# mlozhechko/course5

Measured on AMD Instinct MI355X. Metric: Mrays/sec at 2400x1800 on 1M-tet grid, higher is better.
Workload: dtype f64

## Files before the change

### course5_amd/build.py

```python
from __future__ import annotations

import os
import shutil
import subprocess
import sys

PKG = os.path.dirname(os.path.abspath(__file__))
CSRC = os.path.join(PKG, "csrc")
OUT = os.path.join(PKG, "_build")
LIB = os.path.join(PKG, "libcourse5_hip.so")
CLI = os.path.join(PKG, "course")
ARCH = "gfx950"

HIPCC = shutil.which("hipcc") or "/opt/rocm/bin/hipcc"
COMMON = ["-O3", "-std=c++17", "-fPIC", f"--offload-arch={ARCH}", "-Wall", "-Wextra",
          "-Wno-unused-parameter", "-I", os.path.join(PKG, "..", "include")]

LIB_SOURCES = [
    ("exact_kernels.hip", ["-ffp-contract=off"]),
    ("walk_kernels.hip", []),
    ("adjoint_kernels.hip", ["-munsafe-fp-atomics"]),
    ("context.hip", []),
    ("grid.hip", []),
    ("frame.hip", []),
    ("derivatives.hip", []),
    ("host_ring.hip", []),
    ("adjacency.cpp", ["-x", "c++", "-fopenmp"]),
]


DEVICE_SOURCES = ("device_types.hpp", "kernels.hpp", "walk_common.hpp", "exact_kernels.hip", "walk_kernels.hip")


def kernel_source_hash() -> str:
    import hashlib
    import re
    h = hashlib.sha256()
    for name in DEVICE_SOURCES:
        with open(os.path.join(CSRC, name)) as f:
            text = f.read()
        text = re.sub(r"/\*.*?\*/", "", text, flags=re.S)
        text = re.sub(r"//[^\n]*", "", text)
        h.update(name.encode())
        h.update("".join(text.split()).encode())
    return h.hexdigest()[:16]


def _newer(target: str, deps: list[str]) -> bool:
    if not os.path.exists(target):
        return True
    t = os.path.getmtime(target)
    return any(os.path.getmtime(d) > t for d in deps if os.path.exists(d))


def _run(cmd: list[str], verbose: bool) -> None:
    if verbose:
        print(" ".join(cmd), flush=True)
    subprocess.run(cmd, check=True)


def build_library(verbose: bool = False, force: bool = False) -> str:
    os.makedirs(OUT, exist_ok=True)
    headers = [os.path.join(CSRC, h) for h in os.listdir(CSRC) if h.endswith((".hpp", ".h"))]
    headers.append(os.path.join(PKG, "..", "include", "course5_hip.h"))
    objs = []
    for src, extra in LIB_SOURCES:
        s = os.path.join(CSRC, src)
        o = os.path.join(OUT, os.path.splitext(src)[0] + ".o")
        if force or _newer(o, [s] + headers):
            _run([HIPCC] + COMMON + extra + ["-c", s, "-o", o], verbose)
        objs.append(o)
    if force or _newer(LIB, objs):
        _run([HIPCC, "-shared", "-fPIC", f"--offload-arch={ARCH}", "-o", LIB] + objs + ["-fopenmp"], verbose)
# ... 26 lines not shown
```

### course5_amd/csrc/context.hip

```cpp
#include "context.hpp"

namespace c5api __attribute__((visibility("hidden"))) {

namespace {
std::string g_create_error;
}

int fail(c5_context* ctx, int code, const char* fmt, ...) {
    char buf[512];
    va_list ap;
    va_start(ap, fmt);
    vsnprintf(buf, sizeof buf, fmt, ap);
    va_end(ap);
    if (ctx)
        ctx->error = buf;
    else
        g_create_error = buf;
    return code;
}

int bind_device(c5_context* ctx) {
    C5_HIP(ctx, hipSetDevice(ctx->device));
    return C5_OK;
}
// ... 472 lines not shown
    if (!ctx) return fail(nullptr, C5_ERR_INVALID, "null context");
    ctx->alpha_limit = alpha_limit;
    return C5_OK;
}

int c5_set_option(c5_context* ctx, const char* name, double value) {
    if (!ctx || !name) return fail(ctx, C5_ERR_INVALID, "null option");
    const std::string n(name);
    if (n != "row_costs" && n != "stage_timing" && n != "walk_timing") ++ctx->setup_epoch;
    if (n == "tile") {
        if (value < 0 || value > 3) return fail(ctx, C5_ERR_INVALID, "tile must be 0, 1, 2 or 3");
        ctx->tile_shape = static_cast<int>(value);
    } else if (n == "transmittance_cutoff") {
        ctx->t_cutoff = value;
    } else if (n == "pipeline") {
        int rc = bind_device(ctx);
        if (rc) return rc;
        rc = drain(ctx);
        if (rc) return rc;
        if (ctx->n_cells > 0 || ctx->have_image)
            return fail(ctx, C5_ERR_STATE, "set \"pipeline\" before uploading the grid and setting the image");
        ctx->pipeline = static_cast<int>(value) != 0;
    } else if (n == "fuse_setup") {
        ctx->fuse_setup = static_cast<int>(value) != 0;
    } else if (n == "overlap_setup") {
        ctx->overlap_setup = static_cast<int>(value) != 0;
    } else if (n == "cell_order") {
        ctx->cell_order = static_cast<int>(value) != 0;
    } else if (n == "block_cull") {
        ctx->block_cull = static_cast<int>(value) != 0;
    } else if (n == "tile_flags") {
        ctx->tile_flags = static_cast<int>(value) != 0;
    } else if (n == "cost_order") {
        ctx->cost_order = static_cast<int>(value);
    } else if (n == "entry_key") {
        ctx->entry_key = static_cast<int>(value) != 0;
        ctx->overlap_seen = false;
    } else if (n == "stage_slots") {
        if (value != 0 && value != 14 && value != 21) return fail(ctx, C5_ERR_INVALID, "stage_slots must be 0 (per frame), 14 or 21");
        ctx->stage_slots = static_cast<int>(value);
    } else if (n == "solid_interior_faces") {
        ctx->solid_interior_faces = static_cast<int>(value) != 0;
        forget_solid_masks(ctx);
    } else if (n == "view_cache") {
        ctx->view_cache = static_cast<int>(value) != 0;
    } else if (n == "batch_width") {
        if (value != 0 && value != 4 && value != 8) return fail(ctx, C5_ERR_INVALID, "batch_width must be 0 (by the batch), 4 or 8");
        ctx->batch_width = static_cast<int>(value);
    } else if (n == "vertex_merge") {
        ctx->vertex_merge = static_cast<int>(value) != 0;
    } else if (n == "split_tilt_x" || n == "split_tilt_y") {
        if (!(std::fabs(value) < 64.0)) return fail(ctx, C5_ERR_INVALID, "split tilt out of range");
        (n == "split_tilt_x" ? ctx->split_tilt_x : ctx->split_tilt_y) = value;
    } else if (n == "entry_records") {
        ctx->entry_records = static_cast<int>(value) != 0;
    } else if (n == "depth_split") {
        if (value < 0 || value > c5::kMaxSlabs || value != std::floor(value))
            return fail(ctx, C5_ERR_INVALID, "depth_split must be 0 (per frame), 1 (never) or 2..%d slabs", c5::kMaxSlabs);
        ctx->depth_split = static_cast<int>(value);
    } else if (n == "solid_cache") {
        ctx->solid_cache = static_cast<int>(value) != 0;
        forget_solid_masks(ctx);
    } else if (n == "algorithm") {
        if (value != 0 && value != 1) return fail(ctx, C5_ERR_INVALID, "algorithm must be 0 (walk) or 1 (bin_sort_resolve)");
        ctx->algorithm = static_cast<int>(value);
    } else if (n == "lds_stage") {
        ctx->lds_stage = static_cast<int>(value) < 0 ? 0 : (static_cast<int>(value) > 2 ? 2 : static_cast<int>(value));
    } else if (n == "integration") {
        ctx->order = static_cast<int>(value) != 0;
    } else if (n == "entry_pool") {
        if (value < 1 || value > 16777214) return fail(ctx, C5_ERR_INVALID, "entry_pool out of range");
        int rc = drain(ctx);
        if (rc) return rc;
        for (FrameSlot& fs : ctx->slots) {
            fs.entry_capacity = static_cast<int64_t>(value);
            C5_HIP(ctx, fs.pool.ensure(static_cast<size_t>(fs.entry_capacity) * sizeof(c5::Entry)));
        }
    } else if (n == "band_rows") {
        if (value < 0 || value > 4096) return fail(ctx, C5_ERR_INVALID, "band_rows out of range");
        ctx->band_rows = static_cast<int>(value);
    } else if (n == "lds_pad") {
        if (value < 0 || value > 96 * 1024) return fail(ctx, C5_ERR_INVALID, "lds_pad out of range");
        ctx->lds_pad = static_cast<int>(value);
    } else if (n == "xcd_mode") {
        ctx->xcd_mode = static_cast<int>(value) < 0 ? 0 : (static_cast<int>(value) > 2 ? 2 : static_cast<int>(value));
    } else if (n == "row_costs") {
        ctx->row_costs = static_cast<int>(value) != 0;
    } else if (n == "stage_timing") {
        ctx->stage_timing = static_cast<int>(value) != 0;
    } else if (n == "walk_timing") {
        if (!(value >= 0.0 && value <= 1024.0)) return fail(ctx, C5_ERR_INVALID, "walk_timing: 0 (off) or every N-th launch, N <= 1024");
        ctx->walk_timing = static_cast<int>(value);
        ctx->walk_seq = 0;
    } else {
        return fail(ctx, C5_ERR_INVALID, "unknown option '%s'", name);
    }
    return C5_OK;
}

int c5_get_stats(c5_context* ctx, c5_stats* out) {
    if (!ctx || !out) return fail(ctx, C5_ERR_INVALID, "null argument");
    int rc = c5_synchronize(ctx);
    *out = ctx->last;
    return rc;
}

// ... 67 lines not shown
```

### course5_amd/csrc/context.hpp

```cpp
#pragma once
#include <hip/hip_runtime.h>

#include <algorithm>

#include <cfloat>
#include <cmath>
#include <cstdarg>
#include <cstddef>
#include <cstdio>
#include <cstring>
#include <new>
#include <string>
#include <vector>

#include "../../include/course5_hip.h"
#include "adjacency.hpp"
#include "adjoint.hpp"
#include "device_types.hpp"
#include "kernels.hpp"

namespace c5api __attribute__((visibility("hidden"))) {

struct DeviceBuffer {
    void* ptr = nullptr;
    size_t bytes = 0;
    hipError_t ensure(size_t want) {
        if (want <= bytes && ptr) return hipSuccess;
        if (ptr) {
            hipError_t e = hipFree(ptr);
            ptr = nullptr;
            bytes = 0;
            if (e != hipSuccess) return e;
        }
        if (want == 0) return hipSuccess;
        hipError_t e = hipMalloc(&ptr, want);
        if (e == hipSuccess) bytes = want;
        return e;
    }
    void release() {
        if (ptr) (void)hipFree(ptr);
        ptr = nullptr;
        bytes = 0;
    }
    template <class T>
    T* as() const {
        return static_cast<T*>(ptr);
    }
};

struct Solid {
    int64_t n_tets = 0;
    int64_t n_points = 0;
    int64_t n_faces = 0;
    int64_t n_interior = 0;
    double colour = 0.0;
    struct FaceGroup {
        int64_t begin, count;
        double longest;
    };
    std::vector<FaceGroup> groups;
    double centre[3] = {0, 0, 0};
    double radius = 0.0;
    DeviceBuffer raw;
    DeviceBuffer faces;
    DeviceBuffer view[2];
    c5::RotationList rots{};
    DeviceBuffer own_mask;
    c5::RotationList seen_rots{};
    c5::ImageParams seen_im{};
    uint64_t generation = 0, seen_generation = ~uint64_t{0};
    hipStream_t seen_stream = nullptr;
    int unchanged_frames = 0;
    bool own_mask_ready = false;
};

inline bool same_rotations(const c5::RotationList& a, const c5::RotationList& b) {
    if (a.n != b.n) return false;
    for (int k = 0; k < a.n; ++k)
        if (a.axis[k] != b.axis[k] || a.cosv[k] != b.cosv[k] || a.sinv[k] != b.sinv[k] || a.x0[k] != b.x0[k]) return false;
    return true;
}
inline bool same_image(const c5::ImageParams& a, const c5::ImageParams& b) {
    return a.res_x == b.res_x && a.res_y == b.res_y && a.n_local_rows == b.n_local_rows && a.tile_rows == b.tile_rows &&
           a.rank == b.rank && a.world == b.world && a.row_begin == b.row_begin && a.row_count == b.row_count &&
           a.x_min == b.x_min && a.y_min == b.y_min && a.step_x == b.step_x && a.step_y == b.step_y;
}

constexpr int kWalkEventPool = 512;
constexpr size_t kStageChunk = size_t{4} << 20;
constexpr int kFrameSlots = 2;
constexpr int kStickyWords = 3;
constexpr int kStatusWords = 3;
constexpr int64_t kMaxEntryPool = int64_t{16777214} * 64;
constexpr size_t kCountersBytes = sizeof(c5::FrameCounters) * c5::kCounterLines;

struct FrameSlot {
    DeviceBuffer vx, vy, vz, rec, count, head, first, pool, mask, counters, row_cost;
    DeviceBuffer sb;
    long long sb_key = -1;
    int sb_n = 0;
    uint64_t setup_epoch = 0;
    c5::RotationList setup_view{};
    double setup_limit = 0.0;
    int setup_order = 0;
    bool setup_kept = false;
    bool setup_reused = false;
    const c5::FrameCounters* raster_counters = nullptr;
    DeviceBuffer plane_cell, straddle, straddle_count, partials, arrivals;
    DeviceBuffer bfrec;
    uint32_t bf_seq = 0;
    int split_k = 0;
    int64_t split_px = 0, split_tiles = 0, split_cells = 0;
    uint64_t split_seq = 0;
    int setup_split = 1;
    double setup_w[c5::kMaxSlabs + 1] = {};
    double setup_g[2] = {0.0, 0.0};
    int64_t entry_capacity = 0;
    DeviceBuffer tile_flag;
    uint32_t flag_seq = 0;
    int64_t flag_tiles = 0;
    bool flags_valid = false;
    bool head_clean = false;
    c5::FrameCounters* host_counters = nullptr;
    hipEvent_t setup_done = nullptr, walk_done = nullptr;
    bool walk_recorded = false;
    hipEvent_t ev[7] = {nullptr, nullptr, nullptr, nullptr, nullptr, nullptr, nullptr};
};

}

struct c5_context {
    int device = 0;
    hipStream_t stream = nullptr;
    hipStream_t own_stream = nullptr;
    std::string error;

    int64_t n_pts = 0, n_cells = 0, n_bfaces = 0;
    hipStream_t aux_stream = nullptr;
    hipStream_t side_stream = nullptr;
    hipEvent_t fork_ev = nullptr, join_ev = nullptr;
    int fuse_setup = 0;
    int cell_order = 1;
    std::vector<int32_t> cell_perm;
    int block_cull = 1;
    int tile_flags = 1;
    int cost_order = 1;
    uint8_t sb_order[128] = {};
    long long sb_order_key = -1;
    int sb_order_n = 0;
    uint32_t* host_sb = nullptr;
    int entry_key = 1;
    int stage_slots = 0;
    double rays_per_cell = 0.0;
    int solid_cache = 1;
    int view_cache = 1;
    uint64_t setup_epoch = 1;
    int solid_interior_faces = 0;
    int depth_split = 0;
    int entry_records = 1;
    int split_auto_k = 1;
    bool ray_depth_known = false;
    double ray_depth_lo = 0.0, ray_depth_hi = 0.0;
    bool fit_known = false;
    double fit_gx = 0.0, fit_gy = 0.0, fit_entry0 = 0.0, fit_exit0 = 0.0;
    double split_tilt_x = 0.0, split_tilt_y = 0.0;
    double box_lo[3] = {0, 0, 0}, box_hi[3] = {0, 0, 0};
    double alpha_floor = 0.0;
    int overlap_setup = 0;
    c5api::DeviceBuffer px, py, pz, cell_vert, cell_adj, alpha, q, bface, block_sphere;
    double alpha_top = 0.0;
    double edge_max = 0.0;
    double grid_diagonal = 0.0;
    double coord_max = 0.0;
    c5api::FrameSlot slots[c5api::kFrameSlots];
    int64_t frame_index = 0;
    int last_slot = 0;
    void* last_counters = nullptr;
    int row_cost_slot = 0;
    int algorithm = 0;
    bool grid_conforming = true;
    bool overlap_seen = false;
    c5api::DeviceBuffer offs64, scratch64, segs;
    int pipeline = 0;
    c5::RotationList view{};
    c5api::Solid solids[C5_MAX_SOLIDS];

    bool have_image = false;
    double bounds[4] = {0, 0, 0, 0};
    c5::ImageParams im{};
    int cfg_tile_rows = 0, cfg_rank = 0, cfg_world = 1;
    int cfg_row_begin = 0, cfg_row_count = -1;
    c5api::DeviceBuffer xtab, ytab, out, sticky;
    unsigned* host_sticky = nullptr;
    std::vector<double> host_ytab;
    int row_costs = 0;
    bool row_costs_collected = false;

    double alpha_limit = 2.5;
    double t_cutoff = 1e-12;
    int tile_shape = 3;
    int xcd_mode = 2;
    int lds_pad = 0;
    int band_rows = 0;
    int order = 0;
    int lds_stage = 2;
    int stage_timing = 0;
    int walk_timing = 0;
    unsigned walk_seq = 0;

    hipEvent_t walk_a[c5api::kWalkEventPool];
    hipEvent_t walk_b[c5api::kWalkEventPool];
    int walk_used = 0;
    double walk_ms_sum = 0.0;
    int64_t walk_launches = 0;

    struct HostFrame {
        c5api::DeviceBuffer img;
        c5api::DeviceBuffer counters;
        hipEvent_t rendered = nullptr, copied = nullptr;
        unsigned* status = nullptr;
    };
    hipStream_t copy_stream = nullptr;
// ... 15 lines not shown
    c5api::DeviceBuffer adj_grad;
    c5api::DeviceBuffer adj_perm;
    uint64_t grid_serial = 0, adj_perm_serial = ~uint64_t{0};
    unsigned* adj_status = nullptr;
    bool adjoint_pending = false;
    const char* adj_what = "adjoint";

    c5api::DeviceBuffer tan_dir;

    int batch_width = 0;
    c5api::DeviceBuffer bat_dirs;
    c5api::DeviceBuffer bat_grad;
    c5api::DeviceBuffer gn_g;
    c5api::DeviceBuffer gn_spare;
    c5api::DeviceBuffer vtx_face;
    c5api::DeviceBuffer vtx_grad;
    int vertex_merge = 1;
    c5api::DeviceBuffer vtx_vel;
    std::vector<int32_t> host_cell_vert, point_rep;
    c5api::DeviceBuffer deriv_io;
    c5api::DeviceBuffer scal_stats;
    unsigned long long* scal_host = nullptr;
};

namespace c5api __attribute__((visibility("hidden"))) {

int fail(c5_context* ctx, int code, const char* fmt, ...);

#define C5_HIP(ctx, expr)                                                                        \
    do {                                                                                         \
        hipError_t e_ = (expr);                                                                  \
        if (e_ != hipSuccess)                                                                    \
            return fail((ctx), C5_ERR_HIP, "%s failed: %s (%s:%d)", #expr, hipGetErrorString(e_), \
                        __FILE__, __LINE__);                                                     \
    } while (0)

int bind_device(c5_context* ctx);
int to_rotation_list(c5_context* ctx, const c5_rotation* rots, int n, c5::RotationList& out);
void rotate_host(const c5::RotationList& R, double c[3]);
int drain(c5_context* ctx);
int grow_entry_pools(c5_context* ctx, int64_t want);

int ensure_device_perm(c5_context* ctx);

inline int64_t local_pixels(const c5::ImageParams& im) { return static_cast<int64_t>(im.n_local_rows) * im.res_x; }
inline int64_t padded_pixels(const c5::ImageParams& im) { return ((local_pixels(im) + 1023) / 1024) * 1024; }
inline size_t image_bytes(const c5_context* ctx) { return static_cast<size_t>(local_pixels(ctx->im)) * 2 * sizeof(float); }
bool nothing_to_render(const c5_context* ctx);
bool uses_bin_sort(const c5_context* ctx);
double entry_key_slack(const c5_context* ctx);
c5::GridView grid_view(const c5_context* ctx, const FrameSlot& fs);
int enqueue_bin_lists(c5_context* ctx, FrameSlot& fs, const c5::GridView& g, hipStream_t s, c5::FrameCounters* counters, int64_t& total);
int enqueue_solids(c5_context* ctx, FrameSlot& fs, int slot_id, hipStream_t s, c5::SolidTable& table, bool& any_solid);
int enqueue_frame(c5_context* ctx, float2* out_dev, c5::FrameCounters* own_counters = nullptr);
int wait_and_collect(c5_context* ctx);

int finish_adjoint(c5_context* ctx);

}
```

### course5_amd/csrc/derivatives.hip

```cpp
#include "context.hpp"

using namespace c5api;

namespace {

struct DerivativeView {
    bool no_cells = false;
    bool bin_sort = false;
    hipStream_t s = nullptr;
    int64_t n_px = 0, padded = 0;
    const int32_t* perm = nullptr;
    c5::GridView g{};
    const uint32_t* mask = nullptr;
    c5::WalkParams w{};
};

int setup_derivative(c5_context* ctx, DerivativeView& v) {
    if (nothing_to_render(ctx)) return fail(ctx, C5_ERR_STATE, "plane initializer. empty set of objects to render");
    if (!ctx->have_image) return fail(ctx, C5_ERR_STATE, "critical error. empty plane");
    int rc = bind_device(ctx);
    if (rc) return rc;
    FrameSlot& fs = ctx->slots[0];
    hipStream_t s = v.s = ctx->stream;
    const c5::ImageParams& im = ctx->im;
    v.n_px = local_pixels(im);
    const int64_t padded = v.padded = padded_pixels(im);
    if (ctx->n_cells <= 0) {
        v.no_cells = true;
        return C5_OK;
    }
    if (c5::segment_bytes() != c5::adjoint_segment_bytes())
        return fail(ctx, C5_ERR_STATE, "bin_sort_resolve's segment layout differs from the adjoint's");
    if (ctx->pipeline || ctx->overlap_setup) {
        rc = drain(ctx);
        if (rc) return rc;
    }

    C5_HIP(ctx, ctx->adj_counters.ensure(kCountersBytes));
    C5_HIP(ctx, ctx->adj_sticky.ensure(kStickyWords * sizeof(unsigned)));
    if (!ctx->adj_status) C5_HIP(ctx, hipHostMalloc(reinterpret_cast<void**>(&ctx->adj_status), 4 * sizeof(unsigned), hipHostMallocDefault));
    rc = ensure_device_perm(ctx);
    if (rc) return rc;
    v.perm = ctx->cell_perm.empty() ? nullptr : ctx->adj_perm.as<int32_t>();
    c5::FrameCounters* const counters = ctx->adj_counters.as<c5::FrameCounters>();
    C5_HIP(ctx, hipMemsetAsync(ctx->adj_sticky.ptr, 0, kStickyWords * sizeof(unsigned), s));

    c5::GridView& g = v.g = grid_view(ctx, fs);
    fs.setup_epoch = 0;
    fs.setup_kept = false;
    fs.flags_valid = false;

    c5::launch_transform_soa(s, g.px, g.py, g.pz, g.vx, g.vy, g.vz, g.n_pts, ctx->view, counters);
    c5::SolidTable table{};
    bool any_solid = false;
    v.bin_sort = uses_bin_sort(ctx);
    if (v.bin_sort) {
        int64_t total = 0;
        rc = enqueue_bin_lists(ctx, fs, g, s, counters, total);
        if (rc) return rc;
        rc = enqueue_solids(ctx, fs, 0, s, table, any_solid);
        if (rc) return rc;
        v.mask = any_solid ? fs.mask.as<uint32_t>() : nullptr;
    } else {
        const double key_slack = entry_key_slack(ctx);
        c5::launch_build_records(s, g, ctx->alpha_limit, 0);
        if (!fs.head_clean) C5_HIP(ctx, hipMemsetAsync(fs.head.ptr, 0, static_cast<size_t>(padded) * sizeof(c5::EntryHead), s));
        fs.head_clean = false;
        c5::launch_entry_lists(s, g, ctx->xtab.as<double>(), ctx->ytab.as<double>(), im, fs.head.as<c5::EntryHead>(),
                               fs.first.as<c5::Entry>(), fs.pool.as<c5::Entry>(), fs.entry_capacity, counters,
                               ctx->adj_sticky.as<unsigned>(), 0, key_slack);
        rc = enqueue_solids(ctx, fs, 0, s, table, any_solid);
        if (rc) return rc;
        v.mask = any_solid ? fs.mask.as<uint32_t>() : nullptr;
        c5::WalkParams& wp = v.w;
        wp.xrec = g.xrec;
        wp.entry_head = fs.head.as<c5::EntryHead>();
        wp.entry_first = fs.first.as<c5::Entry>();
        wp.entry_pool = fs.pool.as<c5::Entry>();
        wp.pool_capacity = fs.entry_capacity;
        wp.key_slack = key_slack > 0.0 ? key_slack : 0.0;
        wp.mask = v.mask;
        wp.solids = table;
        wp.Xtab = ctx->xtab.as<double>();
        wp.Ytab = ctx->ytab.as<double>();
        wp.im = im;
        wp.max_steps = static_cast<uint32_t>(ctx->n_cells + 64);
        wp.counters = counters;
        wp.sticky = ctx->adj_sticky.as<unsigned>();
    }
    return C5_OK;
}

int commit_derivative(c5_context* ctx, const char* what) {
    FrameSlot& fs = ctx->slots[0];
    hipStream_t s = ctx->stream;
    C5_HIP(ctx, hipGetLastError());
    C5_HIP(ctx, hipMemcpyAsync(ctx->adj_status, &ctx->adj_counters.as<c5::FrameCounters>()->walk_overflow,
                               kStatusWords * sizeof(unsigned), hipMemcpyDeviceToHost, s));
    if (ctx->pipeline) {
        C5_HIP(ctx, hipEventRecord(fs.walk_done, s));
        fs.walk_recorded = true;
    }
    ctx->adjoint_pending = true;
    ctx->adj_what = what;
    return C5_OK;
}

int adjoint_params(c5_context* ctx, const DerivativeView& v, c5::AdjointParams& ap) {
    C5_HIP(ctx, ctx->adj_lambda.ensure(static_cast<size_t>(v.padded) * sizeof(double)));
    ap = c5::AdjointParams{};
    ap.w = v.w;
    ap.lambda = ctx->adj_lambda.as<double>();
    return C5_OK;
}

int adjoint_one(c5_context* ctx, const DerivativeView& v, bool squared, const float2* weights, double* ga_out, double* gq_out) {
    const size_t n_cells = static_cast<size_t>(ctx->n_cells);
    C5_HIP(ctx, ctx->adj_grad.ensure(2 * n_cells * sizeof(double)));
// ... 613 lines not shown
```

### course5_amd/csrc/frame.hip

```cpp
#include "context.hpp"

namespace c5api __attribute__((visibility("hidden"))) {

constexpr double kSplitAlphaFloor = 1e-6;

int enqueue_solids(c5_context* ctx, FrameSlot& fs, int slot_id, hipStream_t s, c5::SolidTable& table, bool& any_solid) {
    const c5::ImageParams& im = ctx->im;
    const int64_t padded = padded_pixels(im);
    any_solid = false;
    for (int k = 0; k < C5_MAX_SOLIDS; ++k) {
        table.colour[k] = ctx->solids[k].colour;
        if (ctx->solids[k].n_tets > 0) any_solid = true;
    }
    table.n_slots = C5_MAX_SOLIDS;
    if (any_solid) {
        C5_HIP(ctx, hipMemsetAsync(fs.mask.ptr, 0, static_cast<size_t>(padded) * sizeof(uint32_t), s));
        for (int k = 0; k < C5_MAX_SOLIDS; ++k) {
            Solid& so = ctx->solids[k];
            if (so.n_tets <= 0) continue;
            const bool same = ctx->solid_cache && !ctx->pipeline && so.seen_stream == s && so.seen_generation == so.generation &&
                              same_rotations(so.seen_rots, so.rots) && same_image(so.seen_im, im);
            so.unchanged_frames = same ? so.unchanged_frames + 1 : 0;
            if (!same) {
                so.own_mask_ready = false;
// ... 130 lines not shown
    fs.host_counters->seg_tiles = static_cast<unsigned long long>(total);
    if (ctx->pipeline) {
        C5_HIP(ctx, hipEventRecord(fs.setup_done, s));
        C5_HIP(ctx, hipStreamWaitEvent(f.main_s, fs.setup_done, 0));
        C5_HIP(ctx, hipEventRecord(fs.walk_done, f.main_s));
        fs.walk_recorded = true;
    }
    note_enqueued(ctx, f);
    return C5_OK;
}

}

bool nothing_to_render(const c5_context* ctx) {
    if (ctx->n_cells > 0) return false;
    for (const Solid& s : ctx->solids)
        if (s.n_tets > 0) return false;
    return true;
}

c5::GridView grid_view(const c5_context* ctx, const FrameSlot& fs) {
    const c5::ImageParams& im = ctx->im;
    c5::GridView g;
    g.n_pts = ctx->n_pts;
    g.n_cells = ctx->n_cells;
    g.n_bfaces = ctx->n_bfaces;
    g.px = ctx->px.as<double>();
    g.py = ctx->py.as<double>();
    g.pz = ctx->pz.as<double>();
    g.vx = fs.vx.as<double>();
    g.vy = fs.vy.as<double>();
    g.vz = fs.vz.as<double>();
    g.cell_vert = ctx->cell_vert.as<int4>();
    g.cell_adj = ctx->cell_adj.as<int4>();
    g.alpha = ctx->alpha.as<double>();
    g.q = ctx->q.as<double>();
    g.bface = ctx->bface.as<uint32_t>();
    g.xrec = fs.rec.as<c5::ExitRecord>();
    g.rot = ctx->view;
    g.block_sphere = (ctx->block_cull && im.n_local_rows > 0 && im.n_local_rows < im.res_y && ctx->block_sphere.ptr) ? ctx->block_sphere.as<double4>() : nullptr;
    if (im.n_local_rows > 0) {
        const int first = c5::global_row_of(im, 0), last = c5::global_row_of(im, im.n_local_rows - 1);
        const double pad = std::fabs(im.step_y);
        const double ya = ctx->host_ytab[static_cast<size_t>(first)], yb = ctx->host_ytab[static_cast<size_t>(last)];
        g.cull_y_lo = std::fmin(ya, yb) - pad;
        g.cull_y_hi = std::fmax(ya, yb) + pad;
    } else {
        g.cull_y_lo = 1.0;
        g.cull_y_hi = -1.0;
    }
    return g;
}

namespace {


bool serial_setup(const c5_context* ctx) { return !ctx->pipeline && !ctx->fuse_setup && !ctx->overlap_setup; }

bool default_walk(const c5_context* ctx) {
    return ctx->tile_shape == 3 && ctx->xcd_mode == 2 && ctx->lds_stage == 2 && ctx->order == 0;
}

int sb_cost_buffer(c5_context* ctx, FrameJob& f) {
    const c5::ImageParams& im = ctx->im;
    FrameSlot& fs = f.fs;
    if (ctx->cost_order && ctx->xcd_mode == 2 && ctx->lds_stage && im.n_local_rows > 0) {
        const int sb_rows = c5::walk_sb_rows(ctx->tile_shape, ctx->band_rows);
        f.n_sb = (im.n_local_rows + sb_rows - 1) / sb_rows;
        if (f.n_sb <= c5::kMaxSbRows) {
            if (!fs.sb.ptr) {
                C5_HIP(ctx, fs.sb.ensure(c5::kMaxSbRows * sizeof(uint32_t)));
                C5_HIP(ctx, hipMemsetAsync(fs.sb.ptr, 0, fs.sb.bytes, f.s));
            }
            f.sb_key = (static_cast<long long>(im.n_local_rows) << 20) ^ (static_cast<long long>(sb_rows) << 4) ^ ctx->tile_shape;
            f.sb = fs.sb.as<uint32_t>();
        } else {
            f.n_sb = 0;
        }
    }
    fs.sb_key = f.sb_key;
    fs.sb_n = f.n_sb;
    return C5_OK;
}

struct SplitPlan {
    int k = 1;
    double w[c5::kMaxSlabs + 1] = {};
    double g[2] = {0.0, 0.0};
};

void box_depth_range(const c5_context* ctx, const double g[2], double& lo, double& hi) {
    lo = INFINITY, hi = -INFINITY;
    for (int corner = 0; corner < 8; ++corner) {
        double c[3] = {(corner & 1) ? ctx->box_hi[0] : ctx->box_lo[0], (corner & 2) ? ctx->box_hi[1] : ctx->box_lo[1],
                       (corner & 4) ? ctx->box_hi[2] : ctx->box_lo[2]};
        rotate_host(ctx->view, c);
        const double d = c[2] - g[0] * c[0] - g[1] * c[1];
        lo = std::fmin(lo, d);
        hi = std::fmax(hi, d);
    }
}

SplitPlan plan_depth_split(const c5_context* ctx, bool bin_sort) {
    SplitPlan p;
    const bool able = !bin_sort && serial_setup(ctx) && default_walk(ctx) && ctx->n_cells > 0 &&
                      ctx->n_cells < (int64_t{1} << 25) && ctx->im.n_local_rows > 0;
// ... 111 lines not shown
        C5_HIP(ctx, hipMemsetAsync(fs.bfrec.ptr, 0, fs.bfrec.bytes, f.s));
        fs.bf_seq = 0;
    }
    fs.bf_seq += 1;
    if (fs.bf_seq == 0) {
        C5_HIP(ctx, hipMemsetAsync(fs.bfrec.ptr, 0, fs.bfrec.bytes, f.s));
        fs.bf_seq = 1;
    }
    g.bfrec = fs.bfrec.as<c5::BFaceRecord>();
    g.bf_seq = fs.bf_seq;
    g.bf_want_upper = ctx->order != 0;
    g.bf_key_slack = f.key_slack;
    return C5_OK;
}

int tile_flag_buffer(c5_context* ctx, FrameJob& f, const c5::GridView& g, bool fused, hipStream_t e, uint32_t*& tile_flag) {
    FrameSlot& fs = f.fs;
    fs.flags_valid = false;
    if (!(ctx->tile_flags && ctx->tile_shape == 3 && ctx->lds_stage && !fused && g.n_cells > 0 && g.n_bfaces > 0)) return C5_OK;
    const int64_t tiles = c5::walk_tiles(ctx->im);
    if (fs.flag_tiles != tiles || !fs.tile_flag.ptr) {
        C5_HIP(ctx, fs.tile_flag.ensure(static_cast<size_t>(tiles) * sizeof(uint32_t)));
        C5_HIP(ctx, hipMemsetAsync(fs.tile_flag.ptr, 0, static_cast<size_t>(tiles) * sizeof(uint32_t), e));
        fs.flag_tiles = tiles;
        fs.flag_seq = 0;
    }
    fs.flag_seq += 1;
    if (fs.flag_seq == 0) {
        C5_HIP(ctx, hipMemsetAsync(fs.tile_flag.ptr, 0, static_cast<size_t>(tiles) * sizeof(uint32_t), e));
        fs.flag_seq = 1;
    }
    tile_flag = fs.tile_flag.as<uint32_t>();
    fs.flags_valid = true;
    return C5_OK;
}

int enqueue_view_setup(c5_context* ctx, FrameJob& f, c5::GridView& g) {
    FrameSlot& fs = f.fs;
    const c5::ImageParams& im = ctx->im;
    hipStream_t s = f.s;
    const bool side = ctx->overlap_setup && !f.timed;
    hipStream_t e = side ? ctx->side_stream : s;
    if (side) {
        C5_HIP(ctx, hipEventRecord(ctx->fork_ev, s));
        C5_HIP(ctx, hipStreamWaitEvent(e, ctx->fork_ev, 0));
    }
    f.key_slack = entry_key_slack(ctx);
    const bool fused = ctx->fuse_setup && !side && g.n_cells > 0;
    if (!fused && !f.reuse) {
        if (ctx->entry_records && !ctx->fuse_setup && !side && g.n_bfaces > 0) {
            int rc = boundary_records(ctx, f, g);
            if (rc) return rc;
        }
        c5::launch_build_records(s, g, ctx->alpha_limit, ctx->order);
        c5::launch_plane_raster(s, g, ctx->xtab.as<double>(), ctx->ytab.as<double>(), im);
    }
    if (!fused) C5_HIP(ctx, mark(f, 2, s));
    if (!fs.head_clean && !f.reuse) C5_HIP(ctx, hipMemsetAsync(fs.head.ptr, 0, static_cast<size_t>(f.padded) * sizeof(c5::EntryHead), e));
    fs.head_clean = false;
    uint32_t* tile_flag = nullptr;
    if (!f.reuse) {
        int rc = tile_flag_buffer(ctx, f, g, fused, e, tile_flag);
        if (rc) return rc;
    }
    if (fused) {
        c5::launch_setup_fused(s, g, ctx->alpha_limit, ctx->order, ctx->xtab.as<double>(), ctx->ytab.as<double>(), im,
                               fs.head.as<c5::EntryHead>(), fs.first.as<c5::Entry>(), fs.pool.as<c5::Entry>(), fs.entry_capacity,
                               f.counters, ctx->sticky.as<unsigned>(), ctx->order != 0, f.key_slack);
        C5_HIP(ctx, mark(f, 2, s));
    } else if (g.n_cells > 0 && !f.reuse) {
        c5::launch_entry_lists(e, g, ctx->xtab.as<double>(), ctx->ytab.as<double>(), im, fs.head.as<c5::EntryHead>(),
                               fs.first.as<c5::Entry>(), fs.pool.as<c5::Entry>(), fs.entry_capacity, f.counters,
                               ctx->sticky.as<unsigned>(), ctx->order != 0, f.key_slack, tile_flag, fs.flag_seq);
    }
    C5_HIP(ctx, mark(f, 3, e));
    int rc = enqueue_solids(ctx, fs, f.slot_id, e, f.table, f.any_solid);
    if (rc) return rc;
    C5_HIP(ctx, mark(f, 4, e));
    if (side) {
        C5_HIP(ctx, hipEventRecord(ctx->join_ev, e));
        C5_HIP(ctx, hipStreamWaitEvent(s, ctx->join_ev, 0));
    }
    return C5_OK;
}

void fill_walk_params(const c5_context* ctx, const FrameJob& f, const c5::GridView& g, float2* out_dev, c5::WalkParams& wp) {
    const FrameSlot& fs = f.fs;
    wp.xrec = g.xrec;
    wp.entry_head = fs.head.as<c5::EntryHead>();
    wp.entry_first = fs.first.as<c5::Entry>();
    wp.entry_pool = fs.pool.as<c5::Entry>();
    wp.pool_capacity = fs.entry_capacity;
    wp.key_slack = f.key_slack > 0.0 ? f.key_slack : 0.0;
    wp.mask = f.any_solid ? fs.mask.as<uint32_t>() : nullptr;
    wp.solids = f.table;
    wp.Xtab = ctx->xtab.as<double>();
    wp.Ytab = ctx->ytab.as<double>();
    wp.out = out_dev;
    wp.im = ctx->im;
    wp.t_cutoff = ctx->t_cutoff;
    wp.max_steps = static_cast<uint32_t>(ctx->n_cells + 64);
    wp.xcd_mode = ctx->xcd_mode;
    wp.lds_pad = ctx->lds_pad;
    wp.stage_slots = ctx->stage_slots ? ctx->stage_slots : (ctx->rays_per_cell > 0.0 && ctx->rays_per_cell < 120.0 ? 21 : 14);
    wp.band_rows = ctx->band_rows;
    wp.order = ctx->order;
    wp.lds_stage = (ctx->lds_stage && ctx->n_cells < (int64_t{1} << 25)) ? ctx->lds_stage : 0;
    wp.counters = f.counters;
    wp.tile_flag = (fs.flags_valid && !f.any_solid && ctx->tile_flags) ? fs.tile_flag.as<uint32_t>() : nullptr;
    wp.tile_stamp = fs.flag_seq;
    {
        double a_max = std::fmin(ctx->alpha_top, ctx->alpha_limit);
        if (!(a_max >= 0.0)) a_max = ctx->alpha_top;
        wp.small_exp_only = (a_max * ctx->edge_max < 0.125) ? 1 : 0;
    }
    wp.keep_entries = fs.setup_kept ? 1 : 0;
    wp.split = g.split;
    wp.row_cost = nullptr;
    wp.sb_cost = f.sb;
    wp.n_sb_rows = 0;
    if (f.sb && ctx->sb_order_key == f.sb_key && ctx->sb_order_n == f.n_sb) {
// ... 341 lines not shown
```

### course5_amd/csrc/grid.hip

```cpp
#include "context.hpp"

using namespace c5api;

namespace c5api __attribute__((visibility("hidden"))) {

int ensure_device_perm(c5_context* ctx) {
    if (!ctx->cell_perm.empty() && ctx->adj_perm_serial != ctx->grid_serial) {
        const size_t n_cells = static_cast<size_t>(ctx->n_cells);
        C5_HIP(ctx, ctx->adj_perm.ensure(n_cells * sizeof(int32_t)));
        C5_HIP(ctx, hipMemcpy(ctx->adj_perm.ptr, ctx->cell_perm.data(), n_cells * sizeof(int32_t), hipMemcpyHostToDevice));
        ctx->adj_perm_serial = ctx->grid_serial;
    }
    return C5_OK;
}

}

namespace {

void weld_cells(const double* xyz, int64_t n_pts, int64_t n_cells, const int32_t*& cell_vert, std::vector<int32_t>& welded,
                std::vector<int32_t>& rep) {
    if (c5::weld_points(xyz, n_pts, rep) <= 0) {
        rep.clear();
        return;
// ... 123 lines not shown
    for (int64_t i = 0; i < n_pts; ++i)
        for (int k = 0; k < 3; ++k) {
            const double v = xyz[3 * i + k];
            lo[k] = i ? std::fmin(lo[k], v) : v;
            hi[k] = i ? std::fmax(hi[k], v) : v;
            top = std::fmax(top, std::fabs(v));
        }
    for (int k = 0; k < 3; ++k) ctx->box_lo[k] = lo[k], ctx->box_hi[k] = hi[k];
    ctx->grid_diagonal = std::sqrt((hi[0] - lo[0]) * (hi[0] - lo[0]) + (hi[1] - lo[1]) * (hi[1] - lo[1]) + (hi[2] - lo[2]) * (hi[2] - lo[2]));
    ctx->coord_max = top + 2.0;
    double edge2 = 0.0;
    for (int64_t c = 0; c < n_cells; ++c) {
        const int32_t* v = cell_vert + 4 * c;
        for (int a = 0; a < 4; ++a)
            for (int b = a + 1; b < 4; ++b) {
                const double* pa = xyz + 3 * static_cast<int64_t>(v[a]);
                const double* pb = xyz + 3 * static_cast<int64_t>(v[b]);
                const double d2 = (pa[0] - pb[0]) * (pa[0] - pb[0]) + (pa[1] - pb[1]) * (pa[1] - pb[1]) + (pa[2] - pb[2]) * (pa[2] - pb[2]);
                if (d2 > edge2) edge2 = d2;
            }
    }
    ctx->edge_max = std::sqrt(edge2) * (1.0 + 1e-9);
}

int upload_block_spheres(c5_context* ctx, const double* xyz, const int32_t* cell_vert, int64_t n_cells) {
    const int64_t n_blocks = (n_cells + 255) / 256;
    std::vector<double> sph(static_cast<size_t>(4 * n_blocks), 0.0);
    for (int64_t b = 0; b < n_blocks; ++b) {
        double lo[3] = {INFINITY, INFINITY, INFINITY}, hi[3] = {-INFINITY, -INFINITY, -INFINITY};
        for (int64_t c = 256 * b; c < std::min<int64_t>(n_cells, 256 * (b + 1)); ++c)
            for (int a = 0; a < 4; ++a) {
                const double* p = xyz + 3 * static_cast<int64_t>(cell_vert[4 * c + a]);
                for (int k = 0; k < 3; ++k) lo[k] = std::fmin(lo[k], p[k]), hi[k] = std::fmax(hi[k], p[k]);
            }
        double r2 = 0.0;
        for (int k = 0; k < 3; ++k) {
            sph[static_cast<size_t>(4 * b + k)] = 0.5 * (lo[k] + hi[k]);
            r2 += 0.25 * (hi[k] - lo[k]) * (hi[k] - lo[k]);
        }
        sph[static_cast<size_t>(4 * b + 3)] = std::sqrt(r2) * (1.0 + 1e-12);
    }
    C5_HIP(ctx, ctx->block_sphere.ensure(sph.size() * sizeof(double) + 32));
    if (!sph.empty()) C5_HIP(ctx, hipMemcpy(ctx->block_sphere.ptr, sph.data(), sph.size() * sizeof(double), hipMemcpyHostToDevice));
    return C5_OK;
}
}

extern "C" {

int c5_upload_grid(c5_context* ctx, const double* xyz, int64_t n_pts, const int32_t* cell_vert,
                   int64_t n_cells, const double* alpha, const double* q) {
    if (!ctx) return fail(nullptr, C5_ERR_INVALID, "null context");
    ++ctx->setup_epoch;
    if (n_pts < 0 || n_cells < 0) return fail(ctx, C5_ERR_INVALID, "negative size");
    if (n_cells > 0 && (!xyz || !cell_vert || !alpha || !q)) return fail(ctx, C5_ERR_INVALID, "null grid array");
    if (n_cells >= static_cast<int64_t>(c5::kNoCell))
        return fail(ctx, C5_ERR_INVALID, "cell count %lld does not fit 28 bits (line.hpp:71-79)",
                    static_cast<long long>(n_cells));
    for (int64_t i = 0; i < 3 * n_pts; ++i)
        if (!std::isfinite(xyz[i])) return fail(ctx, C5_ERR_INVALID, "point %lld has a non-finite coordinate", static_cast<long long>(i / 3));
    int rc = bind_device(ctx);
    if (rc) return rc;

    for (int64_t i = 0; i < 4 * n_cells; ++i)
        if (cell_vert[i] < 0 || cell_vert[i] >= n_pts)
            return fail(ctx, C5_ERR_INVALID, "cell %lld references a point id out of range", static_cast<long long>(i / 4));
    std::vector<int32_t> welded, ordered;
    std::vector<int32_t> perm;
    std::vector<int32_t> rep;
    weld_cells(xyz, n_pts, n_cells, cell_vert, welded, rep);
    const int32_t* caller_cell_vert = cell_vert;
    if (ctx->cell_order && n_cells >= 4096) morton_order_cells(xyz, n_cells, cell_vert, perm, ordered);
    std::vector<int32_t> adj;
    std::vector<uint32_t> bfaces;
    std::string err;
    bool conforming = true;
    if (!c5::build_face_adjacency(cell_vert, n_cells, n_pts, adj, bfaces, err)) {
        cell_vert = caller_cell_vert;
        perm.clear();
        if (err.find("range") != std::string::npos) return fail(ctx, C5_ERR_INVALID, "%s", err.c_str());
        conforming = false;
        adj.assign(static_cast<size_t>(4 * n_cells), -1);
        bfaces.clear();
    }

    rc = upload_grid_arrays(ctx, xyz, n_pts, cell_vert, n_cells, adj, bfaces, alpha, q, perm);
    if (rc) return rc;
    ctx->cell_perm = std::move(perm);
    ctx->host_cell_vert.assign(cell_vert, cell_vert + 4 * n_cells);
    ctx->point_rep = std::move(rep);
    ++ctx->grid_serial;
    measure_grid(ctx, xyz, n_pts, cell_vert, n_cells);
    scan_alpha(ctx, alpha, n_cells);
    ctx->split_auto_k = 1;
    ctx->ray_depth_known = false;
    ctx->fit_known = false;
    rc = upload_block_spheres(ctx, xyz, cell_vert, n_cells);
    if (rc) return rc;
    ctx->n_pts = n_pts;
    ctx->n_cells = n_cells;
    ctx->n_bfaces = static_cast<int64_t>(bfaces.size());
    ctx->grid_conforming = conforming;
    ctx->overlap_seen = false;
    return C5_OK;
}

int c5_update_scalars(c5_context* ctx, const double* alpha, const double* q, int64_t n_cells) {
    if (!ctx) return fail(nullptr, C5_ERR_INVALID, "null context");
    ++ctx->setup_epoch;
    if (n_cells != ctx->n_cells) return fail(ctx, C5_ERR_INVALID, "scalar count differs from the uploaded grid");
    if (n_cells > 0 && (!alpha || !q)) return fail(ctx, C5_ERR_INVALID, "null scalar array");
    int rc = bind_device(ctx);
    if (rc) return rc;
    C5_HIP(ctx, hipStreamSynchronize(ctx->stream));
    if (n_cells > 0) {
        rc = upload_scalars(ctx, alpha, q, n_cells, ctx->cell_perm);
        if (rc) return rc;
    }
    scan_alpha(ctx, alpha, n_cells);
    return C5_OK;
}

int c5_update_points(c5_context* ctx, const double* xyz, int64_t n_pts) {
    if (!ctx) return fail(nullptr, C5_ERR_INVALID, "null context");
    if (n_pts != ctx->n_pts) return fail(ctx, C5_ERR_INVALID, "point count differs from the uploaded grid");
    if (n_pts > 0 && !xyz) return fail(ctx, C5_ERR_INVALID, "null point array");
    for (int64_t i = 0; i < 3 * n_pts; ++i)
        if (!std::isfinite(xyz[i])) return fail(ctx, C5_ERR_INVALID, "point %lld has a non-finite coordinate", static_cast<long long>(i / 3));
    ++ctx->setup_epoch;
    int rc = bind_device(ctx);
    if (rc) return rc;
    rc = drain(ctx);
    if (rc) return rc;
    std::vector<double> moved;
    if (!ctx->point_rep.empty()) {
        moved.resize(static_cast<size_t>(3 * n_pts));
        for (int64_t i = 0; i < n_pts; ++i)
            for (int k = 0; k < 3; ++k) moved[static_cast<size_t>(3 * i + k)] = xyz[3 * static_cast<int64_t>(ctx->point_rep[static_cast<size_t>(i)]) + k];
        xyz = moved.data();
    }
    std::vector<double> soa(static_cast<size_t>(3 * n_pts));
    for (int64_t i = 0; i < n_pts; ++i)
        for (int k = 0; k < 3; ++k) soa[static_cast<size_t>(k * n_pts + i)] = xyz[3 * i + k];
    const size_t pb = static_cast<size_t>(n_pts) * sizeof(double);
    if (n_pts > 0) {
        C5_HIP(ctx, hipMemcpy(ctx->px.ptr, soa.data(), pb, hipMemcpyHostToDevice));
        C5_HIP(ctx, hipMemcpy(ctx->py.ptr, soa.data() + n_pts, pb, hipMemcpyHostToDevice));
        C5_HIP(ctx, hipMemcpy(ctx->pz.ptr, soa.data() + 2 * n_pts, pb, hipMemcpyHostToDevice));
    }
    const int32_t* cell_vert = ctx->host_cell_vert.data();
    measure_grid(ctx, xyz, n_pts, cell_vert, ctx->n_cells);
    ctx->split_auto_k = 1;
    ctx->ray_depth_known = false;
    ctx->fit_known = false;
    ctx->overlap_seen = false;
    return upload_block_spheres(ctx, xyz, cell_vert, ctx->n_cells);
}

int c5_update_scalars_device(c5_context* ctx, const void* alpha_dev, const void* q_dev, int64_t n_cells) {
    if (!ctx) return fail(nullptr, C5_ERR_INVALID, "null context");
    ++ctx->setup_epoch;
    if (n_cells != ctx->n_cells) return fail(ctx, C5_ERR_INVALID, "scalar count differs from the uploaded grid");
    if (n_cells > 0 && (!alpha_dev || !q_dev)) return fail(ctx, C5_ERR_INVALID, "null scalar array");
    int rc = bind_device(ctx);
    if (rc) return rc;
    if (ctx->pipeline || ctx->overlap_setup) {
        rc = drain(ctx);
        if (rc) return rc;
    }
    double top = 0.0, floor = INFINITY;
    if (n_cells > 0) {
        rc = ensure_device_perm(ctx);
        if (rc) return rc;
        C5_HIP(ctx, ctx->scal_stats.ensure(4 * sizeof(unsigned long long)));
        if (!ctx->scal_host)
            C5_HIP(ctx, hipHostMalloc(reinterpret_cast<void**>(&ctx->scal_host), 4 * sizeof(unsigned long long), hipHostMallocDefault));
        unsigned long long* const stats = ctx->scal_stats.as<unsigned long long>();
        hipStream_t s = ctx->stream;
        C5_HIP(ctx, hipMemsetAsync(stats, 0, 3 * sizeof(unsigned long long), s));
        c5::launch_scalars_gather(s, static_cast<const double*>(alpha_dev), static_cast<const double*>(q_dev),
                                  ctx->cell_perm.empty() ? nullptr : ctx->adj_perm.as<int32_t>(), n_cells, ctx->alpha.as<double>(),
                                  ctx->q.as<double>(), stats);
        C5_HIP(ctx, hipGetLastError());
        C5_HIP(ctx, hipMemcpyAsync(ctx->scal_host, stats, 3 * sizeof(unsigned long long), hipMemcpyDeviceToHost, s));
        C5_HIP(ctx, hipStreamSynchronize(s));
        unsigned long long bits = ctx->scal_host[0];
        std::memcpy(&top, &bits, sizeof top);
        if (ctx->scal_host[2]) {
            floor = 0.0;
        } else if (ctx->scal_host[1]) {
            bits = ~ctx->scal_host[1];
            std::memcpy(&floor, &bits, sizeof floor);
        }
    }
    ctx->alpha_top = top;
    ctx->alpha_floor = floor;
    return C5_OK;
}

}
```

Measured before the change: 8248.

## Split per-cell optics out of record build and cache across frames

Per-cell record building is split into two parts. The optics part depends only on scalars, alpha limit and order; it is written once into units 6-7 of each exit record and rebuilt only when a serial counter shows the scalars changed. Each frame then runs a view-only record kernel that writes the first six units through an LDS-staged, coalesced store, and a fused setup variant uses it too. This cuts per-frame scalar loads and optics arithmetic, at the cost of extra invalidation state and the assumption that the record buffer is not overwritten between frames.

```diff
diff --git a/course5_amd/build.py b/course5_amd/build.py
--- a/course5_amd/build.py
+++ b/course5_amd/build.py
@@ -19,6 +19,7 @@
 LIB_SOURCES = [
     ("exact_kernels.hip", ["-ffp-contract=off"]),
     ("walk_kernels.hip", []),
+    ("record_kernels.hip", []),
     ("adjoint_kernels.hip", ["-munsafe-fp-atomics"]),
     ("context.hip", []),
     ("grid.hip", []),
diff --git a/course5_amd/csrc/context.hip b/course5_amd/csrc/context.hip
--- a/course5_amd/csrc/context.hip
+++ b/course5_amd/csrc/context.hip
@@ -548,6 +548,8 @@
     } else if (n == "split_tilt_x" || n == "split_tilt_y") {
         if (!(std::fabs(value) < 64.0)) return fail(ctx, C5_ERR_INVALID, "split tilt out of range");
         (n == "split_tilt_x" ? ctx->split_tilt_x : ctx->split_tilt_y) = value;
+    } else if (n == "record_optics") {
+        ctx->record_optics = static_cast<int>(value) != 0;
     } else if (n == "entry_records") {
         ctx->entry_records = static_cast<int>(value) != 0;
     } else if (n == "depth_split") {
diff --git a/course5_amd/csrc/context.hpp b/course5_amd/csrc/context.hpp
--- a/course5_amd/csrc/context.hpp
+++ b/course5_amd/csrc/context.hpp
@@ -18,6 +18,7 @@
 #include "adjoint.hpp"
 #include "device_types.hpp"
 #include "kernels.hpp"
+#include "record_kernels.hpp"
 
 namespace c5api __attribute__((visibility("hidden"))) {
 
@@ -105,6 +106,10 @@
     int setup_order = 0;
     bool setup_kept = false;
     bool setup_reused = false;
+    uint64_t optics_serial = 0;
+    uint64_t optics_limit_bits = 0;
+    int optics_order = 0;
+    const void* optics_rec = nullptr;
     const c5::FrameCounters* raster_counters = nullptr;
     DeviceBuffer plane_cell, straddle, straddle_count, partials, arrivals;
     DeviceBuffer bfrec;
@@ -158,6 +163,7 @@
     int solid_interior_faces = 0;
     int depth_split = 0;
     int entry_records = 1;
+    int record_optics = 0;
     int split_auto_k = 1;
     bool ray_depth_known = false;
     double ray_depth_lo = 0.0, ray_depth_hi = 0.0;
@@ -168,6 +174,7 @@
     double alpha_floor = 0.0;
     int overlap_setup = 0;
     c5api::DeviceBuffer px, py, pz, cell_vert, cell_adj, alpha, q, bface, block_sphere;
+    uint64_t scalars_serial = 1;
     double alpha_top = 0.0;
     double edge_max = 0.0;
     double grid_diagonal = 0.0;
@@ -289,6 +296,8 @@
 c5::GridView grid_view(const c5_context* ctx, const FrameSlot& fs);
 int enqueue_bin_lists(c5_context* ctx, FrameSlot& fs, const c5::GridView& g, hipStream_t s, c5::FrameCounters* counters, int64_t& total);
 int enqueue_solids(c5_context* ctx, FrameSlot& fs, int slot_id, hipStream_t s, c5::SolidTable& table, bool& any_solid);
+void ensure_optics(c5_context* ctx, FrameSlot& fs, int order, hipStream_t s);
+void enqueue_records(c5_context* ctx, FrameSlot& fs, const c5::GridView& g, int order, hipStream_t s);
 int enqueue_frame(c5_context* ctx, float2* out_dev, c5::FrameCounters* own_counters = nullptr);
 int wait_and_collect(c5_context* ctx);
 
diff --git a/course5_amd/csrc/derivatives.hip b/course5_amd/csrc/derivatives.hip
--- a/course5_amd/csrc/derivatives.hip
+++ b/course5_amd/csrc/derivatives.hip
@@ -63,7 +63,7 @@
         v.mask = any_solid ? fs.mask.as<uint32_t>() : nullptr;
     } else {
         const double key_slack = entry_key_slack(ctx);
-        c5::launch_build_records(s, g, ctx->alpha_limit, 0);
+        enqueue_records(ctx, fs, g, 0, s);
         if (!fs.head_clean) C5_HIP(ctx, hipMemsetAsync(fs.head.ptr, 0, static_cast<size_t>(padded) * sizeof(c5::EntryHead), s));
         fs.head_clean = false;
         c5::launch_entry_lists(s, g, ctx->xtab.as<double>(), ctx->ytab.as<double>(), im, fs.head.as<c5::EntryHead>(),
diff --git a/course5_amd/csrc/frame.hip b/course5_amd/csrc/frame.hip
--- a/course5_amd/csrc/frame.hip
+++ b/course5_amd/csrc/frame.hip
@@ -206,6 +206,29 @@
     return g;
 }
 
+void ensure_optics(c5_context* ctx, FrameSlot& fs, int order, hipStream_t s) {
+    uint64_t limit_bits;
+    std::memcpy(&limit_bits, &ctx->alpha_limit, sizeof limit_bits);
+    if (fs.optics_serial == ctx->scalars_serial && fs.optics_limit_bits == limit_bits && fs.optics_order == order &&
+        fs.optics_rec == fs.rec.ptr)
+        return;
+    c5::launch_build_optics(s, grid_view(ctx, fs), ctx->alpha_limit, order);
+    fs.optics_serial = ctx->scalars_serial;
+    fs.optics_limit_bits = limit_bits;
+    fs.optics_order = order;
+    fs.optics_rec = fs.rec.ptr;
+}
+
+void enqueue_records(c5_context* ctx, FrameSlot& fs, const c5::GridView& g, int order, hipStream_t s) {
+    if (ctx->record_optics) {
+        fs.optics_serial = 0;
+        c5::launch_build_records(s, g, ctx->alpha_limit, order);
+        return;
+    }
+    ensure_optics(ctx, fs, order, s);
+    c5::launch_build_view_records(s, g, order);
+}
+
 namespace {
 
 
@@ -423,7 +446,7 @@
             int rc = boundary_records(ctx, f, g);
             if (rc) return rc;
         }
-        c5::launch_build_records(s, g, ctx->alpha_limit, ctx->order);
+        enqueue_records(ctx, fs, g, ctx->order, s);
         c5::launch_plane_raster(s, g, ctx->xtab.as<double>(), ctx->ytab.as<double>(), im);
     }
     if (!fused) C5_HIP(ctx, mark(f, 2, s));
@@ -435,9 +458,17 @@
         if (rc) return rc;
     }
     if (fused) {
-        c5::launch_setup_fused(s, g, ctx->alpha_limit, ctx->order, ctx->xtab.as<double>(), ctx->ytab.as<double>(), im,
-                               fs.head.as<c5::EntryHead>(), fs.first.as<c5::Entry>(), fs.pool.as<c5::Entry>(), fs.entry_capacity,
-                               f.counters, ctx->sticky.as<unsigned>(), ctx->order != 0, f.key_slack);
+        if (ctx->record_optics) {
+            fs.optics_serial = 0;
+            c5::launch_setup_fused(s, g, ctx->alpha_limit, ctx->order, ctx->xtab.as<double>(), ctx->ytab.as<double>(), im,
+                                   fs.head.as<c5::EntryHead>(), fs.first.as<c5::Entry>(), fs.pool.as<c5::Entry>(), fs.entry_capacity,
+                                   f.counters, ctx->sticky.as<unsigned>(), ctx->order != 0, f.key_slack);
+        } else {
+            ensure_optics(ctx, fs, ctx->order, s);
+            c5::launch_setup_fused_view(s, g, ctx->order, ctx->xtab.as<double>(), ctx->ytab.as<double>(), im,
+                                        fs.head.as<c5::EntryHead>(), fs.first.as<c5::Entry>(), fs.pool.as<c5::Entry>(), fs.entry_capacity,
+                                        f.counters, ctx->sticky.as<unsigned>(), ctx->order != 0, f.key_slack);
+        }
         C5_HIP(ctx, mark(f, 2, s));
     } else if (g.n_cells > 0 && !f.reuse) {
         c5::launch_entry_lists(e, g, ctx->xtab.as<double>(), ctx->ytab.as<double>(), im, fs.head.as<c5::EntryHead>(),
diff --git a/course5_amd/csrc/grid.hip b/course5_amd/csrc/grid.hip
--- a/course5_amd/csrc/grid.hip
+++ b/course5_amd/csrc/grid.hip
@@ -199,6 +199,7 @@
                    int64_t n_cells, const double* alpha, const double* q) {
     if (!ctx) return fail(nullptr, C5_ERR_INVALID, "null context");
     ++ctx->setup_epoch;
+    ++ctx->scalars_serial;
     if (n_pts < 0 || n_cells < 0) return fail(ctx, C5_ERR_INVALID, "negative size");
     if (n_cells > 0 && (!xyz || !cell_vert || !alpha || !q)) return fail(ctx, C5_ERR_INVALID, "null grid array");
     if (n_cells >= static_cast<int64_t>(c5::kNoCell))
@@ -255,6 +256,7 @@
 int c5_update_scalars(c5_context* ctx, const double* alpha, const double* q, int64_t n_cells) {
     if (!ctx) return fail(nullptr, C5_ERR_INVALID, "null context");
     ++ctx->setup_epoch;
+    ++ctx->scalars_serial;
     if (n_cells != ctx->n_cells) return fail(ctx, C5_ERR_INVALID, "scalar count differs from the uploaded grid");
     if (n_cells > 0 && (!alpha || !q)) return fail(ctx, C5_ERR_INVALID, "null scalar array");
     int rc = bind_device(ctx);
@@ -307,6 +309,7 @@
 int c5_update_scalars_device(c5_context* ctx, const void* alpha_dev, const void* q_dev, int64_t n_cells) {
     if (!ctx) return fail(nullptr, C5_ERR_INVALID, "null context");
     ++ctx->setup_epoch;
+    ++ctx->scalars_serial;
     if (n_cells != ctx->n_cells) return fail(ctx, C5_ERR_INVALID, "scalar count differs from the uploaded grid");
     if (n_cells > 0 && (!alpha_dev || !q_dev)) return fail(ctx, C5_ERR_INVALID, "null scalar array");
     int rc = bind_device(ctx);
diff --git a/course5_amd/csrc/record_kernels.hip b/course5_amd/csrc/record_kernels.hip
--- /dev/null
+++ b/course5_amd/csrc/record_kernels.hip
@@ -0,0 +1,178 @@
+#include <hip/hip_runtime.h>
+
+#include <cfloat>
+
+#include "device_types.hpp"
+#include "record_kernels.hpp"
+#include "walk_common.hpp"
+
+namespace c5 {
+
+namespace {
+
+struct alignas(16) Q4 {
+    uint32_t a, b, c, d;
+};
+constexpr int kRecPad = 9;
+constexpr int kViewUnits = 6;
+__device__ __forceinline__ double plane_tolerance(double coord, double extent) { return 64.0 * DBL_EPSILON * (coord + extent); }
+
+template <bool SPLIT, bool BF>
+__device__ __forceinline__ void view_records_block(const GridView& g, int order, unsigned block, Q4 (*s_rec)[64 * kRecPad]) {
+    const int lane = threadIdx.x & 63, wave = threadIdx.x >> 6;
+    if (g.block_sphere) {
+        const double4 s = g.block_sphere[block];
+        double cx = s.x, cy = s.y, cz = s.z;
+        for (int r = 0; r < g.rot.n; ++r) {
+            const double co = g.rot.cosv[r], si = g.rot.sinv[r];
+            if (g.rot.axis[r] == 0) {
+                const double y_old = cy;
+                cy = cy * co - cz * si;
+                cz = y_old * si + cz * co;
+            } else {
+                cx -= g.rot.x0[r];
+                const double x_old = cx;
+                cx = cx * co - cz * si;
+                cz = x_old * si + cz * co;
+                cx += g.rot.x0[r];
+            }
+        }
+        const double reach = s.w + 1e-9 * (s.w + fabs(cy) + 1.0);
+        if (cy + reach < g.cull_y_lo || cy - reach > g.cull_y_hi) return;
+    }
+    const int64_t cell = block * static_cast<int64_t>(blockDim.x) + threadIdx.x;
+    const int64_t wave_first = cell - lane;
+    bool valid = cell < g.n_cells;
+    CellRecord r;
+    CellOptics o{};
+    double verts[4][3];
+    int4 adj = make_int4(0, 0, 0, 0);
+    if (valid) valid = build_cell_impl<false>(g, 0.0, order, cell, r, o, (SPLIT || BF) ? verts : nullptr, BF ? &adj : nullptr);
+    const unsigned long long valid_mask = __builtin_amdgcn_ballot_w64(valid);
+    if (valid_mask == 0ull) return;
+    if (BF) {
+        const bool b_cell = valid && (adj.x <= -2 || adj.y <= -2 || adj.z <= -2 || adj.w <= -2);
+        if (__builtin_amdgcn_ballot_w64(b_cell) != 0ull && b_cell) {
+            const int nbv[4] = {adj.x, adj.y, adj.z, adj.w};
+#pragma unroll
+            for (int f = 0; f < 4; ++f) {
+                if (nbv[f] > -2) continue;
+                const FacePlane fp = face_plane(verts, f);
+                if (fp.kind == 0 || ((fp.kind > 0) != (g.bf_want_upper != 0))) continue;
+                constexpr int FV3[4][3] = {{0, 1, 2}, {0, 1, 3}, {0, 2, 3}, {1, 2, 3}};
+                const double* a = verts[FV3[f][0]];
+                const double* b = verts[FV3[f][1]];
+                const double* c = verts[FV3[f][2]];
+                BFaceRecord rec;
+                rec.ax = a[0], rec.ay = a[1], rec.bx = b[0], rec.by = b[1], rec.cx = c[0], rec.cy = c[1];
+                rec.x0 = verts[0][0], rec.y0 = verts[0][1];
+                rec.pc = fp.c, rec.pgx = fp.gx, rec.pgy = fp.gy;
+                rec.cell_word = static_cast<uint32_t>(cell) |
+                                (face_key_exponent(a[0], a[1], a[2], b[0], b[1], b[2], c[0], c[1], c[2], fp.gx, fp.gy, g.bf_key_slack) << kEntrySlackShift);
+                rec.seq = g.bf_seq;
+                g.bfrec[-nbv[f] - 2] = rec;
+            }
+        }
+    }
+    if (SPLIT) {
+        double z_lo = 0.0, z_hi = 0.0, tol = 0.0;
+        if (valid) {
+            double d[4], coord = 0.0;
+#pragma unroll
+            for (int k = 0; k < 4; ++k) {
+                d[k] = verts[k][2] - fma(g.split.gx, verts[k][0], g.split.gy * verts[k][1]);
+                coord = fmax(coord, fmax(fabs(verts[k][0]), fmax(fabs(verts[k][1]), fabs(verts[k][2]))));
+            }
+            z_lo = fmin(fmin(d[0], d[1]), fmin(d[2], d[3]));
+            z_hi = fmax(fmax(d[0], d[1]), fmax(d[2], d[3]));
+            tol = plane_tolerance(coord * (1.0 + fabs(g.split.gx) + fabs(g.split.gy)), z_hi - z_lo);
+        }
+        const unsigned shard = static_cast<unsigned>((wave_first >> 6) % kStraddleShards);
+        for (int pl = 1; pl < g.split.n_slabs; ++pl) {
+            const double w = g.split.w[pl];
+            const bool cut = valid && z_lo <= w + tol && z_hi >= w - tol;
+            const unsigned long long cut_mask = __builtin_amdgcn_ballot_w64(cut);
+            if (cut_mask == 0ull) continue;
+            const int leader = __builtin_ctzll(cut_mask);
+            unsigned base = 0;
+            if (lane == leader) base = atomicAdd(g.split.straddle_count + shard * kStraddleCounterStride, static_cast<unsigned>(__popcll(cut_mask)));
+            base = static_cast<unsigned>(__builtin_amdgcn_readlane(static_cast<int>(base), leader));
+            const unsigned at = base + static_cast<unsigned>(__popcll(cut_mask & ((1ull << lane) - 1ull)));
+            if (cut && at < g.split.straddle_capacity)
+                g.split.straddle[static_cast<size_t>(shard) * g.split.straddle_capacity + at] = static_cast<uint32_t>(cell) | (static_cast<uint32_t>(pl - 1) << 28);
+        }
+    }
+    Q4* const my_rec = s_rec[wave];
+    if (valid) {
+        ExitRecord x;
+        to_exit_record(r, o, order, x);
+        const Q4* rp = reinterpret_cast<const Q4*>(&x);
+#pragma unroll
+        for (int k = 0; k < kViewUnits; ++k) my_rec[lane * kRecPad + k] = rp[k];
+    }
+    __builtin_amdgcn_wave_barrier();
+    Q4* const rec_out = reinterpret_cast<Q4*>(g.xrec + wave_first);
+#pragma unroll
+    for (int k = 0; k < 8; ++k) {
+        const int rec_i = k * 8 + (lane >> 3);
+        if (((valid_mask >> rec_i) & 1ull) && (lane & 7) < kViewUnits) rec_out[k * 64 + lane] = my_rec[rec_i * kRecPad + (lane & 7)];
+    }
+}
+
+}
+
+template <bool SPLIT, bool BF>
+__global__ __launch_bounds__(256) void build_view_records(GridView g, int order) {
+    __shared__ Q4 s_rec[4][64 * kRecPad];
+    view_records_block<SPLIT, BF>(g, order, blockIdx.x, s_rec);
+}
+
+__global__ __launch_bounds__(256) void build_optics(GridView g, double alpha_limit, int order) {
+    const int64_t cell = blockIdx.x * static_cast<int64_t>(blockDim.x) + threadIdx.x;
+    if (cell >= g.n_cells) return;
+    const CellOptics o = cell_optics(g, alpha_limit, order, cell);
+    D2* const units = reinterpret_cast<D2*>(g.xrec + cell);
+    units[6] = D2{o.alpha_raw, o.alpha_c};
+    units[7] = D2{o.aux, o.q};
+}
+
+__global__ __launch_bounds__(256) void setup_fused_view(GridView g, int order, unsigned n_rec, unsigned n_ras, RasterArgs A) {
+    __shared__ Q4 s_rec[4][64 * kRecPad];
+    const unsigned b = blockIdx.x, m = n_rec < n_ras ? n_rec : n_ras;
+    const bool raster = b < 2u * m ? (b & 1u) != 0u : n_ras > n_rec;
+    const unsigned idx = b < 2u * m ? b >> 1 : b - m;
+    if (raster)
+        entry_raster_block(g, A, idx);
+    else
+        view_records_block<false, false>(g, order, idx, s_rec);
+}
+
+void launch_build_view_records(hipStream_t s, const GridView& g, int order) {
+    if (g.n_cells <= 0) return;
+    const unsigned blocks = static_cast<unsigned>((g.n_cells + 255) / 256);
+    if (g.split.n_slabs > 1 && g.bfrec)
+        hipLaunchKernelGGL((build_view_records<true, true>), dim3(blocks), dim3(256), 0, s, g, order);
+    else if (g.split.n_slabs > 1)
+        hipLaunchKernelGGL((build_view_records<true, false>), dim3(blocks), dim3(256), 0, s, g, order);
+    else if (g.bfrec)
+        hipLaunchKernelGGL((build_view_records<false, true>), dim3(blocks), dim3(256), 0, s, g, order);
+    else
+        hipLaunchKernelGGL((build_view_records<false, false>), dim3(blocks), dim3(256), 0, s, g, order);
+}
+
+void launch_build_optics(hipStream_t s, const GridView& g, double alpha_limit, int order) {
+    if (g.n_cells <= 0) return;
+    hipLaunchKernelGGL(build_optics, dim3(static_cast<unsigned>((g.n_cells + 255) / 256)), dim3(256), 0, s, g, alpha_limit, order);
+}
+
+void launch_setup_fused_view(hipStream_t s, const GridView& g, int order, const double* Xtab, const double* Ytab,
+                             const ImageParams& im, EntryHead* head, Entry* first, Entry* pool, int64_t capacity,
+                             FrameCounters* counters, unsigned* sticky, int want_upper, double key_slack) {
+    const unsigned n_rec = g.n_cells > 0 ? static_cast<unsigned>((g.n_cells + 255) / 256) : 0u;
+    const unsigned n_ras = g.n_bfaces > 0 ? static_cast<unsigned>((g.n_bfaces + 3) / 4) : 0u;
+    if (n_rec + n_ras == 0u) return;
+    const RasterArgs A{Xtab, Ytab, im, head, first, pool, capacity, counters, sticky, want_upper, key_slack, nullptr, 0u, 0};
+    hipLaunchKernelGGL(setup_fused_view, dim3(n_rec + n_ras), dim3(256), 0, s, g, order, n_rec, n_ras, A);
+}
+
+}
diff --git a/course5_amd/csrc/record_kernels.hpp b/course5_amd/csrc/record_kernels.hpp
--- /dev/null
+++ b/course5_amd/csrc/record_kernels.hpp
@@ -0,0 +1,13 @@
+#pragma once
+
+#include "kernels.hpp"
+
+namespace c5 {
+
+void launch_build_view_records(hipStream_t s, const GridView& g, int order);
+void launch_build_optics(hipStream_t s, const GridView& g, double alpha_limit, int order);
+void launch_setup_fused_view(hipStream_t s, const GridView& g, int order, const double* Xtab, const double* Ytab,
+                             const ImageParams& im, EntryHead* head, Entry* first, Entry* pool, int64_t capacity,
+                             FrameCounters* counters, unsigned* sticky, int want_upper, double key_slack);
+
+}
```

Result: no change. 8328 (median of 6 runs) (+1.0%).
